# ubc-vision/UniT

Measured on AMD Instinct MI355X. Metric: images/sec (fwd+bwd+SGD) R101-C4 VOC 600x1000 bs=2/GPU, higher is better.
Workload: dtype bf16; 1 GPU; UniT base-training step S1 (TrainerNoMeta.run_step): ResNet-101-C4, VOC split1 K=20, 2 supervised + 2 weak 3x600x1000 images per GPU, 512 RoIs/image, two Res5 heads, RPN 12000->2000, all 8 losses, SGD momentum; images_per_gpu=2, global_batch=2, parallelism=dp1

## Files before the change

include/unit_hip.h:

```cpp
#ifndef UNIT_HIP_H
#define UNIT_HIP_H
#include <stddef.h>
#include <stdint.h>
#ifdef __cplusplus
extern "C" {
#endif

int unit_version(void);
const char* unit_build_hash(void);
const char* unit_last_error(void);

int unit_preprocess_image(const float* img_chw, int C, int H, int W, const float* mean3, const float* std3, float prescale,
                          void* out_nhwc, int out_dtype, int Hmax, int Wmax, int Cpad, void* stream);
int unit_resize_u8_pass(const unsigned char* src, int H, int W, int C, int axis, const int* bounds, const int* kk, int ksize,
                        int out_size, unsigned char* dst, void* stream);
int unit_preprocess_u8(const unsigned char* img_hwc, int C, int H, int W, int hflip, const float* mean3, const float* std3,
                       float prescale, void* out_nhwc, int out_dtype, int Hmax, int Wmax, int Cpad, void* stream);
int unit_nchw_to_nhwc(const float* x, void* y, int dtype, int N, int C, int H, int W, int Cp, void* stream);
int unit_nhwc_to_nchw(const void* x, int dtype, float* y, int N, int C, int H, int W, int Cp, void* stream);
int unit_debug_spin(long long cycles, void* sink, void* stream);
int unit_cast(const void* x, int in_dtype, void* y, int out_dtype, long n, void* stream);
int unit_fill_zero(void* p, size_t nbytes, void* stream);
int unit_add_cast(const float* a32, const void* b, const void* mask_ref, void* y, int dtype, long n, void* stream);

// ... 25 lines not shown
                        int N, int H, int W, int C, int K, int R, int S, int stride, int pad, int OH, int OW, int ldy, int oy_mul, int OHf,
                        int OWf, int relu, int tile, int segs, void* stream);
int unit_conv2d_wgrad_x3(const void* x, const void* dy, float* dw, const float* scale_k, int N, int H, int W, int C, int K, int R, int S,
                         int stride, int pad, int OH, int OW, int ldy, int accumulate, int variant, void* workspace, size_t workspace_bytes,
                         void* stream);
int unit_global_avgpool_x3_fwd(const void* y, float* out, int R, int rows, int C, void* stream);
int unit_global_avgpool_x3_bwd_relu(const float* dfeat, const void* y, void* g, int R, int rows, int C, void* stream);
typedef struct UnitConvSecond {
  const void* x; void* y; const void* residual; const void* mask_ref;
  int N, H, W, OHf, OWf;
} UnitConvSecond;
int unit_conv2d_fwd_pair(int kernel, const void* x, const void* w, void* y, const float* bias, const void* residual, const void* mask_ref, int mask_c,
                         int in_dtype, int out_dtype, int N, int H, int W, int C, int K, int R, int S, int stride, int pad, int OH, int OW, int ldy,
                         int oy_mul, int OHf, int OWf, int relu, int tile, const UnitConvSecond* second, void* stream);
size_t unit_conv2d_wgrad_workspace_bytes(int in_dtype, int N, int OH, int OW, int K, int R, int S, int C);
int unit_conv2d_wgrad(const void* x, const void* dy, float* dw, const float* scale_k, int in_dtype, int N, int H, int W, int C,
                      int K, int R, int S, int stride, int pad, int OH, int OW, int ldy, int accumulate, int variant, void* workspace,
                      size_t workspace_bytes, void* stream);
int unit_conv2d_wgrad_splits(int in_dtype, int N, int OH, int OW, int K, int R, int S, int C);
typedef struct UnitWgradProblem {
  const void* x; const void* dy; void* partial;
  int N, H, W, C, K, R, S, stride, pad, OH, OW, ldy;
  int splits, kind;
  int x_pitch;
  int x_back, dy_back;
} UnitWgradProblem;
size_t unit_wgrad_problem_bytes(void);
int unit_conv2d_wgrad_group_supported(int in_dtype, int N, int OH, int OW, int K, int R, int S, int C);
int unit_conv2d_wgrad_group_plan(UnitWgradProblem* pr, int n, int splits_hint);
int unit_conv2d_wgrad_group(const UnitWgradProblem* pr, int n, int in_dtype, void* stream);
int unit_conv2d_wgrad_group_layout(const UnitWgradProblem* pr, int n, int* layout, int layout_rows, int* rows);
int unit_stream_wait_stream(void* waiter, void* signaller);
size_t unit_tensor_desc_bytes(void);
int unit_multi_wgrad_reduce(const void* descs_dev, int n, int total_blocks, float* grads_flat, void* stream);
int unit_multi_weight_prep(const void* descs_dev, int n, int total_blocks, const float* params_flat, int dtype, void* stream);
int unit_shard_sum(const void* parts, int dtype, int nparts, long n, float* out, void* stream);
int unit_comm_unique_id(void* id, int id_bytes);
int unit_comm_init(int rank, int world, const void* id, int id_bytes, void** comm);
int unit_allreduce_bucket_async(void* comm, void* buf, long count, int dtype, void* stream);
int unit_comm_wait(void* compute_stream, void* comm_stream);
int unit_comm_destroy(void* comm);
int unit_comm_rccl_version(void);
int unit_frozen_bn_fold(const float* w, const float* b, const float* rm, const float* rv, float eps, float* scale, float* shift,
                        int C, void* stream);
int unit_weight_prep(const float* w_krsc, const float* scale_k, int K, int R, int S, int C, int Cp, void* w_fwd, void* w_dgrad,
                     int dtype, void* stream);
size_t unit_bias_grad_scratch_bytes(int M, int K);
int unit_bias_grad(const void* dy, int dtype, int M, int K, int ld, float* db, int accumulate, float* scratch, size_t scratch_bytes,
                   void* stream);
size_t unit_linear_wgrad_workspace_bytes(int R, int C, int K);
int unit_linear_wgrad(const void* x, const void* dy, int dtype, int R, int C, int K, int ldy, float* dw, float* db,
                      void* workspace, size_t workspace_bytes, void* stream);
int unit_stem_conv_pool(const void* x, const void* w, const float* shift, void* y, int dtype, int N, int H, int W, void* stream);
int unit_maxpool3x3s2_fwd(const void* x, void* y, int dtype, int N, int H, int W, int C, void* stream);
int unit_global_avgpool_fwd(const void* x, void* y, int dtype, int R, int P, int C, void* stream);
int unit_global_avgpool_bwd_relu(const void* dfeat, const void* out, void* g, int dtype, int R, int P, int C, void* stream);

int unit_anchor_grid(float* out, int H, int W, int A, float stride, float offset, const float* cell_dev, void* stream);

size_t unit_iou_match_workspace_bytes(int B, int Mcap);
int unit_iou_match(const float* gt, const int* gt_count, int B, int Mcap, const float* boxes, long box_batch_stride,
                   const int* box_count, int Ncap, const float* thresholds, const int* labels, int n_thresh,
                   int allow_low_quality, int64_t* match_idx, int8_t* match_label, float* match_val, void* workspace,
                   size_t workspace_bytes, void* stream);
int unit_pairwise_iou(const float* b1, int M, const float* b2, int Nb, float* out, void* stream);
int unit_match_matrix(const float* q, int M, int N, const float* thresholds, const int* labels, int n_thresh, int allow_low_quality,
                      int64_t* match_idx, int8_t* match_label, float* match_val, float* rowmax_ws, void* stream);

int unit_subsample_labels(const void* labels, int labels_are_int64, const int* count, int B, int Ncap, const int* perm, int Pcap,
                          int num_samples, int max_pos, int bg_label, int8_t* out_labels, int* sampled_idx, int* out_counts,
                          void* stream);

int unit_box_encode(const float* src, const float* tgt, const float* weights4, float* out, int n, void* stream);
int unit_box_decode(const float* deltas, int ld, int col0, int K, const float* boxes, const float* weights4, float scale_clamp,
                    float* out, int n, void* stream);

size_t unit_sort_workspace_bytes(int B, int n);
int unit_sort_desc_stable(const float* src, long batch_stride, int ld, int A, int col0, int B, int n, float* out_keys, int* out_idx,
                          void* workspace, size_t workspace_bytes, void* stream);
int unit_sort_desc_stable_topk(const float* src, long batch_stride, int ld, int A, int col0, int B, int n, int topk,
                               float min_exclusive, float* out_keys, int* out_idx, void* workspace, size_t workspace_bytes,
                               void* stream);
int unit_rpn_decode_select(const float* head, long head_batch_stride, int ld, int A, int delta_col0, const float* anchors,
                           const int* sorted_idx, const float* sorted_logit, int B, int Ncap, int topk, const float* image_hw_dev,
                           float scale_clamp, float min_size, float* cand_boxes, float* cand_scores, int* cand_count, void* stream);
size_t unit_nms_workspace_bytes(int B, int cap);
int unit_nms(const float* boxes_sorted, const float* scores_sorted, const int* count, int B, int cap, float thresh, int max_keep,
             int* keep_idx, int* keep_count, float* out_boxes, float* out_scores, void* workspace, size_t workspace_bytes,
             void* stream);

int unit_append_gt(const float* props, const int* pcount, int Pcap, const float* gt, const int* gcount, int Mcap, int B, float* cat,
                   int* ccount, void* stream);
int unit_roi_classes(const int64_t* match_idx, const int8_t* match_label, const int* count, const int64_t* gt_classes,
                     const int* gcount, int Mcap, int B, int Ncap, int K, int64_t* cls, void* stream);
int unit_gather_rois(const float* cat, int Ncap, const int* sampled_idx, int S, const int64_t* cls, const int64_t* match_idx,
                     const float* gt, const int* gcount, int Mcap, int B, float* rois, int* roi_cls, float* roi_gt, void* stream);
int unit_first_k_rois(const float* props, const int* pcount, int Pcap, int S, int B, int batch_index_offset, float* rois, int* valid,
                      void* stream);

int unit_roi_align_fwd(const void* feat_nhwc, int dtype, int N, int H, int W, int C, const float* rois, const int* roi_count_dev,
                       int R, int pooled_size, int out_size, int bin_step, float spatial_scale, int sampling_ratio, int aligned,
                       void* out, void* stream);
int unit_roi_align_bwd(const void* gout, int dtype, int N, int H, int W, int C, const float* rois, const int* roi_count_dev, int R,
                       int pooled_size, int out_size, int bin_step, float spatial_scale, int sampling_ratio, int aligned,
                       float* dfeat_f32, void* stream);

// ... 102 lines not shown
```

unit_amd/build.py:

```python
import hashlib
import os
import subprocess
import sys
from concurrent.futures import ThreadPoolExecutor

HERE = os.path.dirname(os.path.abspath(__file__))
CSRC = os.path.join(HERE, "csrc")
OUT_DIR = os.path.join(HERE, "_build")
LIB = os.path.join(OUT_DIR, "libunit_hip.so")
HEADER = os.path.join(os.path.dirname(HERE), "include", "unit_hip.h")
SOURCES = ["elementwise.hip", "input_pipeline.hip", "boxes.hip", "sort_nms.hip", "roi_align.hip", "losses.hip", "pcl.hip", "conv_igemm.hip", "conv_igemm256.hip", "conv_igemm256p8.hip", "conv_igemm256p8m.hip", "conv_igemm128.hip", "conv_igemm_lc.hip", "conv_wgrad.hip", "conv_wgrad256.hip", "conv_wgrad256p8.hip", "conv_wgrad256r.hip", "conv_wgrad128r.hip", "linear_wgrad.hip", "stem_pool.hip", "detect.hip", "mask.hip", "multi.hip", "split.hip", "comm.hip", "replay.hip"]
STAMP = "build_stamp.hip"
FLAGS = ["--offload-arch=gfx950", "-O3", "-fPIC", "-ffp-contract=off", "-std=c++17", "-Wno-unused-value"]


def _hipcc():
    for c in ("/opt/rocm/bin/hipcc", "hipcc"):
        if os.path.exists(c) or c == "hipcc":
            return c
    return "hipcc"


def _read(path):
    with open(path, "rb") as f:
        return f.read()


def _headers():
    return sorted(os.path.join(CSRC, f) for f in os.listdir(CSRC) if f.endswith(".h"))


def _digest(paths, extra=()):
    h = hashlib.sha256()
    for e in extra:
        h.update(str(e).encode() + b"\0")
    for p in paths:
        h.update(os.path.basename(p).encode() + b"\0")
        h.update(_read(p))
        h.update(b"\0")
    return h.hexdigest()


def source_hash():
    srcs = [os.path.join(CSRC, s) for s in SOURCES + [STAMP]]
    return _digest(srcs + _headers() + [HEADER], extra=FLAGS)


def _stamp_of(path):
    try:
        with open(path + ".hash") as f:
            return f.read().strip()
    except OSError:
        return None


def _write_stamp(path, digest):
    with open(path + ".hash", "w") as f:
        f.write(digest + "\n")


def build(force=False, verbose=False):
    os.makedirs(OUT_DIR, exist_ok=True)
    hdrs = _headers()
    want = source_hash()
# ... 33 lines not shown
```

unit_amd/layers.py:

```python
import os

import torch
from torch import nn

from . import ops


_FROZEN_EPOCH = [0]


def invalidate_prepared():
    _FROZEN_EPOCH[0] += 1


class _EpochOnLoad(nn.Module):
    def _load_from_state_dict(self, *args, **kwargs):
        invalidate_prepared()
        return super()._load_from_state_dict(*args, **kwargs)


def _krsc_storage(w):
    if w.dim() == 2:
        return w if w.is_contiguous() else w.contiguous()
    k, c, r, s = w.shape
# ... 201 lines not shown
            ops.bias_grad(dy_plain.reshape(-1, dy_plain.shape[-1]), self.cout, out=self.bias.grad, accumulate=acc)


def set_x3(module, on):
    n = 0
    for m in module.modules():
        if isinstance(m, Conv2d):
            ok = bool(on) and m.cin % 64 == 0 and m.cout % 64 == 0 and m.cin_pad == m.cin and not getattr(m, "_in_linear_group", False)
            if ok != m.x3:
                m.x3 = ok
                m._prep_key = None
            n += int(ok)
    return n


class BottleneckBlock(nn.Module):

    def __init__(self, cin, cout, bottleneck, stride):
        super().__init__()
        self.stride = stride
        self.shortcut = Conv2d(cin, cout, 1, stride, 0, norm=True) if cin != cout else None
        self.conv1 = Conv2d(cin, bottleneck, 1, stride, 0, norm=True)
        self.conv2 = Conv2d(bottleneck, bottleneck, 3, 1, 1, norm=True)
        self.conv3 = Conv2d(bottleneck, cout, 1, 1, 0, norm=True)

    def convs(self):
        return [c for c in (self.conv1, self.conv2, self.conv3, self.shortcut) if c is not None]

    def fwd(self, x, save=False, stride=None, pool_rows=0, x_bits=None, out_bits=False, pooled_out=None):
        st = self.stride if stride is None else stride
        if isinstance(x, ops.Ragged):
            if self.conv1.x3 and type(x.flat) is not ops.X3:
                x = x.like(ops.x3_split(x.flat))
        elif self.conv1.x3:
            x = ops.as_x3(x)
        y1 = self.conv1.fwd(x, relu=True, stride=st)
        y2 = self.conv2.fwd(y1, relu=True)
        if self._dual_ok(x, y2, st) and not pool_rows:
            wcat, bcat = self._cat_weights("fwd")
            out, bits, _ = ops.conv2d_ex(y2, wcat, self.conv3.cout, 1, 1, 0, bias=bcat, relu=True, want_bits=out_bits, x2=x)
            return ((out, bits) if out_bits else out), ((x, y1, y2, st, x_bits) if save else None)
        sc = self.shortcut.fwd(x, stride=st) if self.shortcut is not None else x
        if pool_rows:
            c3 = self.conv3
            _, bits, pooled = ops.conv2d_ex(y2, c3.wf, c3.cout, 1, 1, 0, bias=c3.shift, residual=sc, relu=True, want_bits=save,
                                            pool_rows=pool_rows, want_y=False, pooled_out=pooled_out)
            return (pooled, bits), ((x, y1, y2, st, x_bits) if save else None)
        if out_bits:
            c3 = self.conv3
            out, bits, _ = ops.conv2d_ex(y2, c3.wf, c3.cout, 1, 1, 0, bias=c3.shift, residual=sc, relu=True, want_bits=True)
            return (out, bits), ((x, y1, y2, st, x_bits) if save else None)
        out = self.conv3.fwd(y2, relu=True, residual=sc)
        return out, ((x, y1, y2, st, x_bits) if save else None)

    def _dual_ok(self, x, y2, st):
        if isinstance(x, ops.Ragged):
            return False
        return (ops.FUSE_EPILOGUE and ops.FUSE_DUAL and getattr(self, "allow_dual", False) and self.shortcut is not None and st == 1
                and x.dtype == torch.bfloat16 and x.shape[:3] == y2.shape[:3] and x.shape[0] > 0
                and ops.conv_ex_supported(x.dtype, self.conv3.cin, self.conv3.cout) and self.shortcut.cin % self.conv3.cin == 0
                and self.shortcut.cout % self.conv1.cout == 0 and self.conv1.cout % 64 == 0 and self.conv1.cin % 64 == 0)

    def prepare_dual(self):
        if not (ops.FUSE_EPILOGUE and ops.FUSE_DUAL and getattr(self, "allow_dual", False) and self.shortcut is not None):
            return
        c3, sc, c1 = self.conv3, self.shortcut, self.conv1
        if c3.x3 or sc.x3 or c1.x3:
            return
        if c3.wf is None or sc.wf is None or c3.wf.dtype != torch.bfloat16 or c3.k != 1 or sc.k != 1 or c1.k != 1:
            return
        key = (c3.wf.data_ptr(), sc.wf.data_ptr(), 0 if c1.wd is None else c1.wd.data_ptr(), 0 if sc.wd is None else sc.wd.data_ptr(),
               0 if c3.shift is None else c3.shift.data_ptr(), 0 if sc.shift is None else sc.shift.data_ptr())
        if self.__dict__.get("_dual_key") == key:
            return
        dev, dt = c3.wf.device, c3.wf.dtype
        buf = torch.empty((c3.cout, 1, 1, c3.cin + sc.cin), dtype=dt, device=dev)
        v = buf.view(c3.cout, -1)
        c3.link_copy("wf", v[:, :c3.cin])
        sc.link_copy("wf", v[:, c3.cin:])
        self.__dict__["_wcat_fwd"] = buf
        self.__dict__["_wcat_bwd"] = None
        if c1.wd is not None and sc.wd is not None:
            bufb = torch.empty((c1.cin, 1, 1, c1.cout + sc.cout), dtype=dt, device=dev)
            vb = bufb.view(c1.cin, -1)
            c1.link_copy("wd", vb[:, :c1.cout])
            sc.link_copy("wd", vb[:, c1.cout:])
            self.__dict__["_wcat_bwd"] = bufb
        self.__dict__["_bcat"] = c3.shift + sc.shift
        self.__dict__["_dual_key"] = key

    def _cat_weights(self, which):
        self.prepare_dual()
        buf = self.__dict__.get("_wcat_" + which)
        assert buf is not None, "dual-input GEMM before the block's weights were prepared"
        return buf, (self.__dict__["_bcat"] if which == "fwd" else None)

    def bwd(self, ctx, g, need_dx=True, mask_input=True):
        x, y1, y2, st, x_bits = ctx
        rag = isinstance(x, ops.Ragged)
        if rag:
            if self.conv3.x3 and type(g.flat) is not ops.X3:
                g = g.like(ops.x3_split(g.flat))
        elif self.conv3.x3:
            g = ops.as_x3(g)
        hw_of = (lambda t: t.dims) if rag else (lambda t: t.shape[1:3])
        self.conv3.wgrad(y2, g)
        dy2 = self.conv3.dgrad(g, hw_of(y2), mask_ref=y2)
        self.conv2.wgrad(y1, dy2)
        dy1 = self.conv2.dgrad(dy2, hw_of(y1), mask_ref=y1)
        self.conv1.wgrad(x, dy1, stride=st)
        if self.shortcut is not None:
            self.shortcut.wgrad(x, g, stride=st)
        if not need_dx:
            return None
        hw = hw_of(x)
        if self._dual_ok(x, y2, st) and not mask_input and g.dtype == torch.bfloat16:
            wcat, _ = self._cat_weights("bwd")
            return ops.conv2d_ex(dy1, wcat, self.conv1.cin, 1, 1, 0, x2=g)[0]
        if self.shortcut is not None:
            dsc = self.shortcut.dgrad(g, hw, stride=st)
        else:
            dsc = g
        return self.conv1.dgrad(dy1, hw, mask_ref=x if mask_input else None, residual=dsc, stride=st, mask_bits=x_bits if mask_input else None)


class ResStage(nn.Sequential):
    def __init__(self, num_blocks, cin, cout, bottleneck, first_stride):
        blocks = [BottleneckBlock(cin if i == 0 else cout, cout, bottleneck, first_stride if i == 0 else 1) for i in range(num_blocks)]
        super().__init__(*blocks)

    def fwd(self, x, save=False, first_stride=None, pool_rows=0, out_bits=False, pooled_out=None):
        ctxs = []
        x_bits = None
        for i, b in enumerate(self):
            last = i == len(self) - 1
            ob = (out_bits and not last and not isinstance(x, ops.Ragged) and ops.conv_ex_supported(x.dtype, b.conv3.cin, b.conv3.cout)
                  and (i > 0 or (first_stride or b.stride) == 1))
            x, c = b.fwd(x, save, stride=first_stride if i == 0 else None, pool_rows=pool_rows if last else 0, x_bits=x_bits, out_bits=ob,
                         pooled_out=pooled_out if last else None)
            x_bits = None
            if ob:
                x, x_bits = x
            ctxs.append(c)
        return x, ctxs

    def bwd(self, ctxs, g, need_dx=True, mask_input=True, on_block_done=None):
        n = len(self)
        for i in range(n - 1, -1, -1):
            first = i == 0
            g = self[i].bwd(ctxs[i], g, need_dx=(need_dx or not first), mask_input=(mask_input or not first))
            if on_block_done is not None:
                on_block_done(i)
        return g

    BUCKET_BLOCKS = 6

    def bucket_of_block(self, i):
        n = len(self)
        if n <= self.BUCKET_BLOCKS + 2:
            return 0
        return (n - 1 - i) // self.BUCKET_BLOCKS

    def last_block_of_bucket(self, k):
        n = len(self)
        if n <= self.BUCKET_BLOCKS + 2:
            return 0
        return max(0, n - (k + 1) * self.BUCKET_BLOCKS)


_FUSED_STEM = os.environ.get("UNIT_FUSED_STEM", "1") != "0"


class BasicStem(nn.Module):

    def __init__(self, cout=64):
        super().__init__()
        self.conv1 = Conv2d(3, cout, 7, 2, 3, norm=True, cin_pad=8)

    def fwd(self, x):
        c = self.conv1
        if isinstance(x, (list, tuple)):
            dims = []
            for t in x:
                n, h, w, _ = t.shape
                oh, ow = (h - 1) // 2 + 1, (w - 1) // 2 + 1
                dims.append((n, (oh - 1) // 2 + 1, (ow - 1) // 2 + 1))
            out = ops.Ragged.empty(dims, c.cout, x[0])
            for i, t in enumerate(x):
                self._fwd_one(t, out.group(i))
            return out
        return self._fwd_one(x, None)

    def _fwd_one(self, x, out):
        c = self.conv1
        if (_FUSED_STEM and x.dtype == torch.bfloat16 and x.is_cuda and c.cout == 64 and x.shape[-1] == 8 and c.wf is not None
                and c.wf.dtype == torch.bfloat16 and not c.weight.requires_grad):
            return ops.stem_conv_pool(x, c.wf, c.shift, out=out)
# ... 122 lines not shown
```

unit_amd/modeling/backbone.py:

```python
import os

import torch
from torch import nn

from .. import ops
from ..layers import BasicStem, ResStage
from ..structures import BACKBONE_REGISTRY, ShapeSpec

BLOCKS = {50: [3, 4, 6, 3], 101: [3, 4, 23, 3], 152: [3, 8, 36, 3]}


class ResNet(nn.Module):
    def __init__(self, depth=101, freeze_at=2, res2_out=256, width=64):
        super().__init__()
        nb = BLOCKS[depth]
        self.depth = depth
        self.stem = BasicStem(64)
        self.res2 = ResStage(nb[0], 64, res2_out, width, 1)
        self.res3 = ResStage(nb[1], res2_out, res2_out * 2, width * 2, 2)
        self.res4 = ResStage(nb[2], res2_out * 2, res2_out * 4, width * 4, 2)
        self.out_channels = res2_out * 4
        self.size_divisibility = 0
        self.freeze_at = freeze_at
        self.freeze(freeze_at)

    def freeze(self, freeze_at):
        stages = [self.stem, self.res2, self.res3, self.res4]
        for i, s in enumerate(stages, start=1):
            if freeze_at >= i:
                for p in s.parameters():
                    p.requires_grad = False
        self.res2[0].allow_dual = freeze_at >= 2 and os.environ.get("UNIT_RES2_DUAL", "0") == "1"
        return self

    def output_shape(self):
        return {"res4": ShapeSpec(channels=self.out_channels, stride=16)}

    def all_convs(self):
        cs = [self.stem.conv1]
        for st in (self.res2, self.res3, self.res4):
            for b in st:
                cs += b.convs()
        return cs

    def prepare(self, dtype, version):
        for c in self.all_convs():
            c.prepare(dtype, version, need_dgrad=c.weight.requires_grad)

    def first_trainable_stage(self):
        for i, st in enumerate((self.res2, self.res3, self.res4)):
            if any(p.requires_grad for p in st.parameters()):
                return i
        return 3

    def fwd(self, x, save=False, before_trainable=None):
        joined = False
        if before_trainable is not None and any(p.requires_grad for p in self.stem.parameters()):
            before_trainable()
            joined = True
        x = self.stem.fwd(x)
        ft = self.first_trainable_stage()
        ctx = []
        for i, st in enumerate((self.res2, self.res3, self.res4)):
            if i == ft and before_trainable is not None and not joined:
                before_trainable()
            x, c = st.fwd(x, save=save and i >= ft)
            ctx.append(c)
        return x, ctx

    def bwd(self, ctx, g, on_stage_done=None):
        ft = self.first_trainable_stage()
        stages = (self.res2, self.res3, self.res4)
        for i in (2, 1, 0):
            if i < ft:
                break
            name, st = ("res2", "res3", "res4")[i], stages[i]
            cb = None
            if on_stage_done is not None:
                def cb(j, name=name, st=st):
                    k = st.bucket_of_block(j)
                    if j == st.last_block_of_bucket(k):
                        on_stage_done(name if k == 0 else f"{name}.{k}")
            g = st.bwd(ctx[i], g, need_dx=(i > ft), mask_input=True, on_block_done=cb)
        return None

    def forward(self, x):
        if self.training and torch.is_grad_enabled():
            from .train_modules import backbone_forward_train
            return backbone_forward_train(self, x)
        dtype = getattr(self, "compute_dtype", torch.bfloat16)
        self.prepare(dtype, 0)
        xh = ops.nchw_to_nhwc(x, dtype=dtype, cpad=8)
        y, _ = self.fwd(xh)
        return {"res4": ops.nhwc_to_nchw(y)}


@BACKBONE_REGISTRY.register()
def build_resnet_backbone(cfg, input_shape=None):
    r = cfg.MODEL.RESNETS
    assert r.NORM == "FrozenBN" and r.STRIDE_IN_1X1 and r.NUM_GROUPS == 1, "C4 hot path: FrozenBN, stride_in_1x1, groups=1"
    assert list(r.OUT_FEATURES) == ["res4"]
    return ResNet(r.DEPTH, cfg.MODEL.BACKBONE.FREEZE_AT, r.RES2_OUT_CHANNELS, r.WIDTH_PER_GROUP)
```

unit_amd/ops.py:

```python
import ctypes
import os
import math

import torch

from ._lib import _DEBUG_SYNC, check, lib

F32, BF16 = 0, 1
SCALE_CLAMP = math.log(1000.0 / 16)


def dt(dtype):
    if dtype == torch.float32:
        return F32
    if dtype == torch.bfloat16:
        return BF16
    raise TypeError(f"unsupported dtype {dtype}")


def _p(t):
    if t is None:
        return None
    if not t.is_cuda:
        raise RuntimeError("unit_amd ops need tensors on the ROCm device (no CPU fallback)")
# ... 352 lines not shown
            out = zeros((n, ohf, owf, ldy), out_dtype, x.device)
        else:
            out = torch.empty((n, ohf, owf, ldy), dtype=out_dtype, device=x.device)
    prof = PROFILER
    if prof is not None:
        e0 = torch.cuda.Event(enable_timing=True)
        e0.record()
    big, mid, variant = False, -1, 0
    if tile_cfg == 0:
        pkey = (x.dtype, n * oh * ow, k, c, r * s * c, out_dtype, ldy % 8, BIG_TILE_POLICY, MID_TILE_POLICY)
        pol = _POLICY_CACHE.get(pkey)
        if pol is None:
            pol = _POLICY_CACHE[pkey] = select_conv_kernel(x.dtype, n * oh * ow, k, c, r * s * c, out_dtype, ldy)
        big, mid = pol
    elif tile_cfg >= 100:
        mid = tile_cfg
    elif tile_cfg in TILE_CFG:
        kind, code = TILE_CFG[tile_cfg]
        if kind == "big":
            big, variant = True, code
        else:
            mid = code
    if mid >= 0:
        check(lib().unit_conv2d_fwd_mid(_p(x), _p(w), _p(out), _p(bias), _p(residual), _p(mask_ref), dt(out_dtype),
                                        n, h, wd, c, k, r, s, stride, pad, oh, ow, ldy, oy_mul, ohf, owf, int(relu), mid, _s()),
              "unit_conv2d_fwd_mid")
    elif big:
        check(lib().unit_conv2d_fwd_big(_p(x), _p(w), _p(out), _p(bias), _p(residual), _p(mask_ref), dt(out_dtype),
                                        n, h, wd, c, k, r, s, stride, pad, oh, ow, ldy, oy_mul, ohf, owf, int(relu),
                                        variant, _s()),
              "unit_conv2d_fwd_big")
    else:
        check(lib().unit_conv2d_fwd(_p(x), _p(w), _p(out), _p(bias), _p(residual), _p(mask_ref), dt(x.dtype), dt(out_dtype),
                                    n, h, wd, c, k, r, s, stride, pad, oh, ow, ldy, oy_mul, ohf, owf, int(relu), tile_cfg, _s()),
              "unit_conv2d_fwd")
    if prof is not None:
        e1 = torch.cuda.Event(enable_timing=True)
        e1.record()
        es = out.element_size()
        nbytes = (x.numel() + w.numel()) * x.element_size() + n * oh * ow * ldy * es * (1 + (residual is not None) + (mask_ref is not None))
        feed = None
        if mid >= 0:
            bm, bn = mid_tile_dims(mid)
            tiles = ((n * oh * ow + bm - 1) // bm) * ((k + bn - 1) // bn)
            feed = ((tiles + 255) // 256) * (r * s * c // 64) * (bm + bn) * 128.0
        prof.setdefault("conv_igemm256" if (big and mid < 0) else ("conv_igemm_dma" if mid >= 0 else "conv_igemm"), []).append(
            (e0, e1, 2.0 * n * oh * ow * k * r * s * c, nbytes, feed))
    return out


FUSE_EPILOGUE = os.environ.get("UNIT_FUSE_EPILOGUE", "1") != "0"


FUSE_DUAL = os.environ.get("UNIT_FUSE_DUAL", "1") != "0"


def conv_ex_supported(dtype, c, ldy):
    return dtype == torch.bfloat16 and c % 64 == 0 and ldy % 64 == 0


class ReluBits:

    def __init__(self, data, r, bins, c, roi0=0):
        self.data, self.r, self.bins, self.c, self.roi0 = data, r, bins, c, roi0

    def __getitem__(self, sl):
        start, stop, step = sl.indices(self.r)
        assert step == 1
        return ReluBits(self.data, stop - start, self.bins, self.c, self.roi0 + start)

    def aligned(self):
        m0 = self.roi0 * self.bins
        if m0 % 128:
            return None
        return self if m0 == 0 else ReluBits(self.data[(m0 // 128) * (self.c // 64) * 1024:], self.r, self.bins, self.c, 0)

    def unpack(self):
        dev = self.data.device
        m = torch.arange(self.roi0 * self.bins, (self.roi0 + self.r) * self.bins, device=dev).view(-1, 1)
        n = torch.arange(self.c, device=dev).view(1, -1)
        word = ((m >> 7) * (self.c >> 6) + (n >> 6)) * 64 + ((m & 7) * 8 + ((n & 63) >> 3))
        byte = self.data[word * 16 + ((m & 127) >> 3)]
        return ((byte.int() >> (n & 7)) & 1).bool().view(self.r, self.bins, self.c)


def conv2d_ex(x, w, k, r, s, pad=0, bias=None, residual=None, relu=False, mask_bits=None, want_bits=False, pool_rows=0, want_y=True, x2=None, variant=0,
              pooled_out=None):
    n, h, wd, c = x.shape
    c2 = 0
    if x2 is not None:
        c2 = x2.shape[3]
        assert r == 1 and s == 1 and pad == 0 and x2.shape[:3] == x.shape[:3] and c2 % c == 0 and x2.dtype == x.dtype and w.shape[-1] == c + c2
    oh, ow = conv_out_size(h, wd, r, s, 1, pad)
    ldy = k
    assert conv_ex_supported(x.dtype, c, ldy), "conv2d_ex: bf16, C % 64 == 0, K % 8 == 0"
    m = n * oh * ow
    y = torch.empty((n, oh, ow, ldy), dtype=x.dtype, device=x.device) if want_y else None
    bits = None
    if want_bits:
        bits = ReluBits(torch.empty(lib().unit_relu_bits_bytes(m, ldy), dtype=torch.uint8, device=x.device), n, oh * ow, k)
    if mask_bits is not None:
        assert mask_bits.roi0 == 0 and mask_bits.r * mask_bits.bins == m and mask_bits.c == k
    part = None
    if pool_rows:
        assert pool_rows == oh * ow
        part = torch.empty(lib().unit_conv_pool_partial_floats(m, ldy), dtype=torch.float32, device=x.device)
# ... 417 lines not shown
def frozen_bn_fold(weight, bias, running_mean, running_var, eps=1e-5):
    c = weight.numel()
    scale = torch.empty(c, dtype=torch.float32, device=weight.device)
    shift = torch.empty(c, dtype=torch.float32, device=weight.device)
    check(lib().unit_frozen_bn_fold(_p(weight), _p(bias), _p(running_mean), _p(running_var), eps, _p(scale), _p(shift), c, _s()),
          "frozen_bn_fold")
    return scale, shift


def weight_prep(w_krsc, scale, k, r, s, c, cp, dtype, want_dgrad=True, w_fwd=None, w_dgrad=None):
    dev = w_krsc.device
    if w_fwd is None:
        w_fwd = torch.empty((k, r, s, cp), dtype=dtype, device=dev)
    if want_dgrad and w_dgrad is None:
        w_dgrad = torch.empty((c, r, s, k), dtype=dtype, device=dev)
    check(lib().unit_weight_prep(_p(w_krsc), _p(scale), k, r, s, c, cp, _p(w_fwd), _p(w_dgrad) if want_dgrad else None,
                                 dt(dtype), _s()), "weight_prep")
    return w_fwd, w_dgrad


def bias_grad(dy2d, k, out=None, accumulate=False):
    m, ld = dy2d.shape
    if out is None:
        out = torch.empty(k, dtype=torch.float32, device=dy2d.device)
    nb = lib().unit_bias_grad_scratch_bytes(m, k) if m > 1024 else 0
    ws = workspace(nb, dy2d.device, slot=3) if nb else None
    check(lib().unit_bias_grad(_p(dy2d), dt(dy2d.dtype), m, k, ld, _p(out), int(accumulate), _p(ws), nb, _s()), "bias_grad")
    return out


def linear_wgrad(x2d, dy2d, k, dw, db):
    r, c = x2d.shape
    ldy = dy2d.shape[1]
    dev = x2d.device
    nb = lib().unit_linear_wgrad_workspace_bytes(r, c, k)
    ws = workspace(nb, dev, slot=4)
    with _timed("conv_wgrad", 2.0 * r * k * c, (x2d.numel() + r * ldy) * 2 + 4 * k * c):
        check(lib().unit_linear_wgrad(_p(x2d), _p(dy2d), dt(x2d.dtype), r, c, k, ldy, _p(dw), _p(db), _p(ws), ws.numel(), _s()),
              "unit_linear_wgrad")


def stem_conv_pool(x, w_fwd, shift, out=None):
    n, h, w, c = x.shape
    assert c == 8 and tuple(w_fwd.shape) == (64, 7, 7, 8) and x.dtype == torch.bfloat16 and w_fwd.dtype == torch.bfloat16
    oh, ow = (h - 1) // 2 + 1, (w - 1) // 2 + 1
    ph, pw = (oh - 1) // 2 + 1, (ow - 1) // 2 + 1
    y = out if out is not None else torch.empty((n, ph, pw, 64), dtype=x.dtype, device=x.device)
    assert tuple(y.shape) == (n, ph, pw, 64) and y.is_contiguous()
    with _timed("stem", 2.0 * n * oh * ow * 64 * 147, x.numel() * 2 + y.numel() * 2):
        check(lib().unit_stem_conv_pool(_p(x), _p(w_fwd), _p(shift), _p(y), dt(x.dtype), n, h, w, _s()), "unit_stem_conv_pool")
    return y


def maxpool3x3s2(x, out=None):
    n, h, w, c = x.shape
    oh, ow = (h + 2 - 3) // 2 + 1, (w + 2 - 3) // 2 + 1
    y = out if out is not None else torch.empty((n, oh, ow, c), dtype=x.dtype, device=x.device)
    assert tuple(y.shape) == (n, oh, ow, c) and y.is_contiguous() and y.dtype == x.dtype
    check(lib().unit_maxpool3x3s2_fwd(_p(x), _p(y), dt(x.dtype), n, h, w, c, _s()), "maxpool")
    return y


def global_avgpool(x, out=None):
    r, ph, pw, c = x.shape
    if out is not None:
        assert out.shape == (r, c) and out.is_contiguous() and out.dtype == (torch.float32 if type(x) is X3 else x.dtype)
    if type(x) is X3:
        y = out if out is not None else torch.empty((r, c), dtype=torch.float32, device=x.device)
        check(lib().unit_global_avgpool_x3_fwd(_px(x), _p(y), r, ph * pw, c, _s()), "avgpool_x3_fwd")
        return y
    y = out if out is not None else torch.empty((r, c), dtype=x.dtype, device=x.device)
    check(lib().unit_global_avgpool_fwd(_p(x), _p(y), dt(x.dtype), r, ph * pw, c, _s()), "avgpool_fwd")
    return y


def global_avgpool_bwd_relu(dfeat, out):
    r, ph, pw, c = out.shape
    if type(out) is X3:
        g = torch.empty(out.shape, dtype=torch.float32, device=out.device).as_subclass(X3)
        check(lib().unit_global_avgpool_x3_bwd_relu(_p(dfeat), _px(out), _px(g), r, ph * pw, c, _s()), "avgpool_x3_bwd")
        return g
    g = torch.empty_like(out)
    check(lib().unit_global_avgpool_bwd_relu(_p(dfeat), _p(out), _p(g), dt(out.dtype), r, ph * pw, c, _s()), "avgpool_bwd")
    return g


def cell_anchors(sizes=(32, 64, 128, 256, 512), ratios=(0.5, 1.0, 2.0)):
    out = []
    for size in sizes:
        area = size ** 2.0
        for r in ratios:
            w = math.sqrt(area / r)
            h = r * w
            out.append([-w / 2.0, -h / 2.0, w / 2.0, h / 2.0])
    return torch.tensor(out, dtype=torch.float32)


def anchor_grid(h, w, cell, stride=16, offset=0.0):
    a = cell.shape[0]
    out = torch.empty((h * w * a, 4), dtype=torch.float32, device=cell.device)
    check(lib().unit_anchor_grid(_p(out), h, w, a, float(stride), float(offset), _p(cell), _s()), "anchor_grid")
    return out


def iou_match(gt, gt_count, boxes, box_count, thresholds, labels, allow_low_quality, want_vals=True):
    b, mcap = gt.shape[0], gt.shape[1]
# ... 452 lines not shown
```

Baseline: 132.6 images/sec.

## Fuse frozen res2 bottleneck blocks into one persistent HIP kernel

Adds a kernel that runs a whole frozen res2 bottleneck block (1x1, 3x3, 1x1, plus the optional shortcut conv, with bias, residual and ReLU) per spatial tile in LDS. Weights stay in registers, and the next tile is prefetched with buffer-load-to-LDS. When the next stage begins with a stride-2 1x1 conv, the last block writes only the pixels that consumer reads. This removes the intermediate activation round-trips to HBM and the per-conv launches in the frozen res2 stage. In exchange it recomputes halo pixels for conv1, and the stride-2 output leaves the other pixels unwritten, so correctness depends on no other consumer reading them.

Measured after the change: 131.6 images/sec, median of 2. Within noise of the previous version (-0.7%).

```diff
diff --git a/include/unit_hip.h b/include/unit_hip.h
--- a/include/unit_hip.h
+++ b/include/unit_hip.h
@@ -101,6 +101,8 @@
 int unit_linear_wgrad(const void* x, const void* dy, int dtype, int R, int C, int K, int ldy, float* dw, float* db,
                       void* workspace, size_t workspace_bytes, void* stream);
 int unit_stem_conv_pool(const void* x, const void* w, const float* shift, void* y, int dtype, int N, int H, int W, void* stream);
+int unit_res2_block_fwd(const void* x, const void* w1, const float* b1, const void* w2, const float* b2, const void* w3, const float* b3,
+                        const void* wsc, const float* bsc, void* y, int N, int H, int W, int cin, int out_stride, void* stream);
 int unit_maxpool3x3s2_fwd(const void* x, void* y, int dtype, int N, int H, int W, int C, void* stream);
 int unit_global_avgpool_fwd(const void* x, void* y, int dtype, int R, int P, int C, void* stream);
 int unit_global_avgpool_bwd_relu(const void* dfeat, const void* out, void* g, int dtype, int R, int P, int C, void* stream);
diff --git a/unit_amd/build.py b/unit_amd/build.py
--- a/unit_amd/build.py
+++ b/unit_amd/build.py
@@ -9,7 +9,7 @@
 OUT_DIR = os.path.join(HERE, "_build")
 LIB = os.path.join(OUT_DIR, "libunit_hip.so")
 HEADER = os.path.join(os.path.dirname(HERE), "include", "unit_hip.h")
-SOURCES = ["elementwise.hip", "input_pipeline.hip", "boxes.hip", "sort_nms.hip", "roi_align.hip", "losses.hip", "pcl.hip", "conv_igemm.hip", "conv_igemm256.hip", "conv_igemm256p8.hip", "conv_igemm256p8m.hip", "conv_igemm128.hip", "conv_igemm_lc.hip", "conv_wgrad.hip", "conv_wgrad256.hip", "conv_wgrad256p8.hip", "conv_wgrad256r.hip", "conv_wgrad128r.hip", "linear_wgrad.hip", "stem_pool.hip", "detect.hip", "mask.hip", "multi.hip", "split.hip", "comm.hip", "replay.hip"]
+SOURCES = ["elementwise.hip", "input_pipeline.hip", "boxes.hip", "sort_nms.hip", "roi_align.hip", "losses.hip", "pcl.hip", "conv_igemm.hip", "conv_igemm256.hip", "conv_igemm256p8.hip", "conv_igemm256p8m.hip", "conv_igemm128.hip", "conv_igemm_lc.hip", "conv_wgrad.hip", "conv_wgrad256.hip", "conv_wgrad256p8.hip", "conv_wgrad256r.hip", "conv_wgrad128r.hip", "linear_wgrad.hip", "stem_pool.hip", "res2_block.hip", "detect.hip", "mask.hip", "multi.hip", "split.hip", "comm.hip", "replay.hip"]
 STAMP = "build_stamp.hip"
 FLAGS = ["--offload-arch=gfx950", "-O3", "-fPIC", "-ffp-contract=off", "-std=c++17", "-Wno-unused-value"]
 
diff --git a/unit_amd/csrc/res2_block.hip b/unit_amd/csrc/res2_block.hip
--- /dev/null
+++ b/unit_amd/csrc/res2_block.hip
@@ -0,0 +1,314 @@
+#include "common.h"
+#include "conv_epilogue.h"
+#ifndef UNIT_RES2_DBG
+#define UNIT_RES2_DBG 0
+#endif
+
+namespace {
+
+typedef __attribute__((address_space(3))) void lds_void_r;
+
+constexpr int TH = 4, TW = 16;
+constexpr int NW = 4;
+constexpr int NA = 256 / NW / 16;
+constexpr int PW = TW + 2;
+constexpr int PPIX = (TH + 2) * PW;
+constexpr int PROWS = (PPIX + 15) / 16 * 16;
+constexpr int PBLK = PROWS / 16, PPIECES = PROWS / 8;
+constexpr int PLANE = PROWS * 128;
+constexpr int Y2_BYTES = TH * TW * 128;
+constexpr int OPLANE_SC = TH * TW * 128;
+
+template <bool SC> struct Lds {
+  static constexpr int NPL = SC ? 1 : 4;
+  static constexpr int Y1 = NPL * PLANE, Y2 = Y1 + PLANE;
+  static constexpr int OUT = SC ? Y2 + Y2_BYTES : 0;
+  static constexpr int SHIFT = SC ? OUT + 4 * OPLANE_SC : Y2 + Y2_BYTES;
+  static constexpr int BYTES = SHIFT + (SC ? 2048 : 1024);
+};
+static_assert(2 * Lds<true>::BYTES <= 160 * 1024 && 2 * Lds<false>::BYTES <= 160 * 1024, "LDS budget: two workgroups per CU");
+
+struct Res2Args {
+  const bf16_t* x; const bf16_t* w1; const bf16_t* w2; const bf16_t* w3; const bf16_t* wsc;
+  const float* b1; const float* b2; const float* b3; const float* bsc;
+  bf16_t* y;
+  int N, H, W, tiles_x, tiles_y, ntiles, per_xcd;
+  unsigned x_bytes;
+};
+
+__device__ __forceinline__ int swz_r(int row, int chunk) { return row * 128 + ((chunk ^ ((row >> 1) & 7)) << 4); }
+
+__device__ __forceinline__ bf16x8 ldw(const bf16_t* w, int row, int pitch, int k) {
+  return __builtin_bit_cast(bf16x8, *reinterpret_cast<const i32x4*>(w + (size_t)row * pitch + k));
+}
+
+template <bool RELU, bool RES>
+__device__ __forceinline__ i32x2 finish4(const f32x4& acc, const float (&b)[4], i32x2 res) {
+  float v[4];
+#pragma unroll
+  for (int j = 0; j < 4; ++j) v[j] = acc[j] + b[j];
+  if constexpr (RES) {
+    v[0] += epi_lo((unsigned)res[0]); v[1] += epi_hi((unsigned)res[0]);
+    v[2] += epi_lo((unsigned)res[1]); v[3] += epi_hi((unsigned)res[1]);
+  }
+  unsigned o0 = epi_cvt_pk(v[0], v[1]), o1 = epi_cvt_pk(v[2], v[3]);
+  if constexpr (RELU) { o0 = epi_relu_pk(o0); o1 = epi_relu_pk(o1); }
+  return i32x2{(int)o0, (int)o1};
+}
+
+template <bool SC, int OS>
+__global__ void __launch_bounds__(NW * 64, 2) res2_block_kernel(Res2Args p) {
+  typedef Lds<SC> L;
+  constexpr int CIN = SC ? 64 : 256;
+  constexpr int KS1 = CIN / 32;
+  constexpr int NPT = TH * TW / (OS * OS) / 16;
+  constexpr int NCP = NPT * 16 * 32 / (NW * 64);
+  extern __shared__ __attribute__((aligned(16))) char smem[];
+  char* const xs = smem;
+  char* const y1 = smem + L::Y1;
+  char* const y2 = smem + L::Y2;
+  char* const outs = smem + L::OUT;
+  float* const shifts = reinterpret_cast<float*>(smem + L::SHIFT);
+
+  const int tid = threadIdx.x, lane = tid & 63;
+  const int wid = __builtin_amdgcn_readfirstlane(tid >> 6);
+  const int frow = lane & 15, fq = lane >> 4;
+  const int sl = wid;
+  const int lrow = lane >> 3, lc = lane & 7;
+
+  __amdgpu_buffer_rsrc_t rsX = __builtin_amdgcn_make_buffer_rsrc(const_cast<bf16_t*>(p.x), 0, (int)p.x_bytes, 0x00020000);
+  constexpr unsigned OOB = 0xFFFFFFF0u;
+
+  const int xcd = blockIdx.x & 7, loc0 = blockIdx.x >> 3, wg_per_xcd = gridDim.x >> 3;
+  auto tile_of = [&](int loc) { int t = xcd * p.per_xcd + loc; return (loc < p.per_xcd && t < p.ntiles) ? t : -1; };
+
+  bool staged = false;
+  auto stage = [&](int tile) {
+    int tx = tile % p.tiles_x, t2 = tile / p.tiles_x, ty = t2 % p.tiles_y, n = t2 / p.tiles_y;
+    int py0 = ty * TH - 1, px0 = tx * TW - 1;
+    if ((UNIT_RES2_DBG & 1) && staged) return;
+    staged = true;
+#pragma unroll
+    for (int i = 0; i < (L::NPL * PPIECES + NW - 1) / NW; ++i) {
+      int pc = wid + NW * i;
+      if (pc >= L::NPL * PPIECES) break;
+      int pl = pc / PPIECES, R0 = (pc - pl * PPIECES) * 8;
+      int row = R0 + lrow;
+      int q = lc ^ ((row >> 1) & 7);
+      int py = row / PW, px = row - py * PW;
+      int yy = py0 + py, xx = px0 + px;
+      bool ok = row < PPIX && (unsigned)yy < (unsigned)p.H && (unsigned)xx < (unsigned)p.W;
+      unsigned off = ((unsigned)((n * p.H + yy) * p.W + xx) * (unsigned)CIN + (unsigned)(pl * 64 + q * 8)) * 2u;
+      __builtin_amdgcn_raw_ptr_buffer_load_lds(rsX, (lds_void_r*)(xs + pl * PLANE + R0 * 128), 16, ok ? off : OOB, 0, 0, 0);
+    }
+  };
+
+  int loc = loc0;
+  int tile = tile_of(loc);
+  if (tile >= 0) stage(tile);
+
+  bf16x8 fw1[KS1], fw2[9][2], fw3[NA][2], fws[SC ? NA : 1][2];
+  float bb1[4], bb2[4];
+  static_assert(NW * 64 == 256, "one thread per output channel");
+  shifts[tid] = p.b3[tid];
+  if constexpr (SC) shifts[256 + tid] = p.bsc[tid];
+#pragma unroll
+  for (int j = 0; j < KS1; ++j) fw1[j] = ldw(p.w1, sl * 16 + frow, CIN, j * 32 + fq * 8);
+#pragma unroll
+  for (int t = 0; t < 9; ++t)
+#pragma unroll
+    for (int ks = 0; ks < 2; ++ks) fw2[t][ks] = ldw(p.w2, sl * 16 + frow, 576, t * 64 + ks * 32 + fq * 8);
+#pragma unroll
+  for (int a = 0; a < NA; ++a)
+#pragma unroll
+    for (int ks = 0; ks < 2; ++ks) {
+      fw3[a][ks] = ldw(p.w3, wid * (NA * 16) + a * 16 + frow, 64, ks * 32 + fq * 8);
+      if constexpr (SC) fws[a][ks] = ldw(p.wsc, wid * (NA * 16) + a * 16 + frow, 64, ks * 32 + fq * 8);
+    }
+#pragma unroll
+  for (int j = 0; j < 4; ++j) {
+    bb1[j] = p.b1[sl * 16 + fq * 4 + j];
+    bb2[j] = p.b2[sl * 16 + fq * 4 + j];
+  }
+  auto shift4 = [&](const float* b, int a, float (&v)[4]) {
+    f32x4 t = *reinterpret_cast<const f32x4*>(b + wid * (NA * 16) + a * 16 + fq * 4);
+    v[0] = t[0]; v[1] = t[1]; v[2] = t[2]; v[3] = t[3];
+  };
+
+  auto out_pos = [](int j, int& py, int& px) {
+    if constexpr (OS == 1) { py = j >> 4; px = j & 15; }
+    else { py = (j >> 3) * 2; px = (j & 7) * 2; }
+  };
+
+  while (tile >= 0) {
+    const int tx = tile % p.tiles_x, t2 = tile / p.tiles_x, ty = t2 % p.tiles_y, n = t2 / p.tiles_y;
+    const int y0 = ty * TH, x0 = tx * TW;
+    asm volatile("s_waitcnt vmcnt(0)" ::: "memory");
+    __syncthreads();
+
+    if (!(UNIT_RES2_DBG & 2)) {
+#pragma unroll 1
+    for (int rt = 0; rt < PBLK; ++rt) {
+      const int row = rt * 16 + frow;
+      f32x4 acc = {0.f, 0.f, 0.f, 0.f};
+      bf16x8 fx[KS1];
+#pragma unroll
+      for (int j = 0; j < KS1; ++j) fx[j] = *reinterpret_cast<const bf16x8*>(xs + (j >> 1) * PLANE + swz_r(row, (j & 1) * 4 + fq));
+#pragma unroll
+      for (int j = 0; j < KS1; ++j) acc = __builtin_amdgcn_mfma_f32_16x16x32_bf16(fw1[j], fx[j], acc, 0, 0, 0);
+      int py = row / PW, px = row - py * PW;
+      bool in_map = row < PPIX && (unsigned)(y0 - 1 + py) < (unsigned)p.H && (unsigned)(x0 - 1 + px) < (unsigned)p.W;
+      i32x2 o = finish4<true, false>(acc, bb1, i32x2{0, 0});
+      if (!in_map) o = i32x2{0, 0};
+      const int ch = sl * 16 + fq * 4;
+      *reinterpret_cast<i32x2*>(y1 + swz_r(row, ch >> 3) + (ch & 4) * 2) = o;
+    }
+    }
+    __syncthreads();
+
+    if (!(UNIT_RES2_DBG & 2)) {
+#pragma unroll 1
+    for (int i = 0; i < NPT; ++i) {
+      const int j0 = i * 16;
+      int py, px;
+      out_pos(j0 + frow, py, px);
+      f32x4 acc = {0.f, 0.f, 0.f, 0.f};
+#pragma unroll
+      for (int r = 0; r < 3; ++r) {
+        bf16x8 fx[3][2];
+#pragma unroll
+        for (int s = 0; s < 3; ++s)
+#pragma unroll
+          for (int ks = 0; ks < 2; ++ks) fx[s][ks] = *reinterpret_cast<const bf16x8*>(y1 + swz_r((py + r) * PW + px + s, ks * 4 + fq));
+#pragma unroll
+        for (int s = 0; s < 3; ++s)
+#pragma unroll
+          for (int ks = 0; ks < 2; ++ks) acc = __builtin_amdgcn_mfma_f32_16x16x32_bf16(fw2[r * 3 + s][ks], fx[s][ks], acc, 0, 0, 0);
+      }
+      i32x2 o = finish4<true, false>(acc, bb2, i32x2{0, 0});
+      const int ch = sl * 16 + fq * 4;
+      *reinterpret_cast<i32x2*>(y2 + swz_r(j0 + frow, ch >> 3) + (ch & 4) * 2) = o;
+    }
+    }
+    __syncthreads();
+
+    if (!(UNIT_RES2_DBG & 2)) {
+#pragma unroll 1
+    for (int pt = 0; pt < NPT; ++pt) {
+      const int j = pt * 16 + frow;
+      int py, px;
+      out_pos(j, py, px);
+      const int prow = (py + 1) * PW + px + 1;
+      bf16x8 f2[2];
+#pragma unroll
+      for (int ks = 0; ks < 2; ++ks) f2[ks] = *reinterpret_cast<const bf16x8*>(y2 + swz_r(j, ks * 4 + fq));
+      f32x4 acc[NA];
+#pragma unroll
+      for (int a = 0; a < NA; ++a) acc[a] = f32x4{0.f, 0.f, 0.f, 0.f};
+#pragma unroll
+      for (int a = 0; a < NA; ++a)
+#pragma unroll
+        for (int ks = 0; ks < 2; ++ks) acc[a] = __builtin_amdgcn_mfma_f32_16x16x32_bf16(fw3[a][ks], f2[ks], acc[a], 0, 0, 0);
+      i32x2 res[NA];
+      if constexpr (SC) {
+        bf16x8 fxs[2];
+#pragma unroll
+        for (int ks = 0; ks < 2; ++ks) fxs[ks] = *reinterpret_cast<const bf16x8*>(xs + swz_r(prow, ks * 4 + fq));
+#pragma unroll
+        for (int a = 0; a < NA; ++a) {
+          f32x4 as = {0.f, 0.f, 0.f, 0.f};
+#pragma unroll
+          for (int ks = 0; ks < 2; ++ks) as = __builtin_amdgcn_mfma_f32_16x16x32_bf16(fws[a][ks], fxs[ks], as, 0, 0, 0);
+          float bs[4];
+          shift4(shifts + 256, a, bs);
+          res[a] = finish4<false, false>(as, bs, i32x2{0, 0});
+        }
+      }
+#pragma unroll
+      for (int a = 0; a < NA; ++a) {
+        const int ch = wid * (NA * 16) + a * 16 + fq * 4;
+        const int orow = SC ? j : prow;
+        char* q = outs + (ch >> 6) * (SC ? OPLANE_SC : PLANE) + swz_r(orow, (ch & 63) >> 3) + (ch & 4) * 2;
+        if constexpr (!SC) res[a] = *reinterpret_cast<const i32x2*>(q);
+        float b3[4];
+        shift4(shifts, a, b3);
+        *reinterpret_cast<i32x2*>(q) = finish4<true, true>(acc[a], b3, res[a]);
+      }
+    }
+    }
+    __syncthreads();
+
+    loc += wg_per_xcd;
+    const int next = tile_of(loc);
+    constexpr int NH = NCP / 2;
+    i32x4 ov[NH];
+    auto take = [&](int k0) {
+#pragma unroll
+      for (int k = 0; k < NH; ++k) {
+        int item = tid + NW * 64 * (k0 + k);
+        int j = item >> 5, c = item & 31;
+        int py, px;
+        out_pos(j, py, px);
+        const int orow = SC ? j : (py + 1) * PW + px + 1;
+        ov[k] = *reinterpret_cast<const i32x4*>(outs + (c >> 3) * (SC ? OPLANE_SC : PLANE) + swz_r(orow, c & 7));
+      }
+    };
+    auto put = [&](int k0) {
+#pragma unroll
+      for (int k = 0; k < NH; ++k) {
+        int item = tid + NW * 64 * (k0 + k);
+        int j = item >> 5, c = item & 31;
+        int py, px;
+        out_pos(j, py, px);
+        int yy = y0 + py, xx = x0 + px;
+        if (yy < p.H && xx < p.W && (!(UNIT_RES2_DBG & 4) || ov[k][0] == 0x7fc17fc3))
+          *reinterpret_cast<i32x4*>(p.y + (((size_t)n * p.H + yy) * p.W + xx) * 256 + c * 8) = ov[k];
+      }
+    };
+    take(0);
+    put(0);
+    take(NH);
+    if constexpr (!SC) __syncthreads();
+    if (next >= 0) stage(next);
+    put(NH);
+    tile = next;
+  }
+}
+
+template <bool SC, int OS>
+int launch_res2(const Res2Args& a, hipStream_t st) {
+  static bool attr_set = false;
+  if (!attr_set) {
+    (void)hipFuncSetAttribute((const void*)res2_block_kernel<SC, OS>, hipFuncAttributeMaxDynamicSharedMemorySize, Lds<SC>::BYTES);
+    attr_set = true;
+  }
+  int grid = a.ntiles < 512 ? (a.ntiles + 7) / 8 * 8 : 512;
+  res2_block_kernel<SC, OS><<<grid, NW * 64, Lds<SC>::BYTES, st>>>(a);
+  UNIT_LAUNCH_CHECK();
+  return UNIT_OK;
+}
+
+}
+
+extern "C" int unit_res2_block_fwd(const void* x, const void* w1, const float* b1, const void* w2, const float* b2, const void* w3,
+                                   const float* b3, const void* wsc, const float* bsc, void* y, int N, int H, int W, int cin, int out_stride,
+                                   void* stream) {
+  UNIT_CHECK_ARG(x && w1 && b1 && w2 && b2 && w3 && b3 && y, "unit_res2_block_fwd: null tensor");
+  UNIT_CHECK_ARG((wsc != nullptr) == (bsc != nullptr), "unit_res2_block_fwd: shortcut weights and shift come together");
+  UNIT_CHECK_ARG(cin == (wsc ? 64 : 256), "unit_res2_block_fwd: 64 input channels with a shortcut conv, 256 without");
+  UNIT_CHECK_ARG(out_stride == 1 || out_stride == 2, "unit_res2_block_fwd: out_stride must be 1 or 2");
+  UNIT_CHECK_ARG(N > 0 && H > 0 && W > 0 && (size_t)N * H * W * 256 * 2 < 0xFFFFFFF0ull, "unit_res2_block_fwd: bad shape");
+  UNIT_CHECK_ARG(((uintptr_t)x % 16 == 0) && ((uintptr_t)y % 16 == 0) && ((uintptr_t)w1 % 16 == 0) && ((uintptr_t)w2 % 16 == 0) &&
+                 ((uintptr_t)w3 % 16 == 0) && ((uintptr_t)wsc % 16 == 0), "unit_res2_block_fwd: 16B alignment");
+  Res2Args a;
+  a.x = (const bf16_t*)x; a.w1 = (const bf16_t*)w1; a.w2 = (const bf16_t*)w2; a.w3 = (const bf16_t*)w3; a.wsc = (const bf16_t*)wsc;
+  a.b1 = b1; a.b2 = b2; a.b3 = b3; a.bsc = bsc; a.y = (bf16_t*)y;
+  a.N = N; a.H = H; a.W = W;
+  a.tiles_x = cdiv(W, TW); a.tiles_y = cdiv(H, TH);
+  a.ntiles = a.tiles_x * a.tiles_y * N;
+  a.per_xcd = cdiv(a.ntiles, 8);
+  a.x_bytes = (unsigned)((size_t)N * H * W * cin * 2);
+  hipStream_t st = (hipStream_t)stream;
+  if (wsc) return out_stride == 1 ? launch_res2<true, 1>(a, st) : launch_res2<true, 2>(a, st);
+  return out_stride == 1 ? launch_res2<false, 1>(a, st) : launch_res2<false, 2>(a, st);
+}
diff --git a/unit_amd/layers.py b/unit_amd/layers.py
--- a/unit_amd/layers.py
+++ b/unit_amd/layers.py
@@ -277,6 +277,21 @@
             return (out, bits), ((x, y1, y2, st, x_bits) if save else None)
         out = self.conv3.fwd(y2, relu=True, residual=sc)
         return out, ((x, y1, y2, st, x_bits) if save else None)
+
+    def fused_frozen_ok(self, cin):
+        c1, c2, c3, sc = self.conv1, self.conv2, self.conv3, self.shortcut
+        if self.stride != 1 or getattr(self, "allow_dual", False) or any(p.requires_grad for p in self.parameters()):
+            return False
+        if any(c.x3 or c.wf is None or c.wf.dtype != torch.bfloat16 or c.shift is None or c.cin_pad != c.cin for c in self.convs()):
+            return False
+        if (c1.k, c1.cin, c1.cout, c2.k, c2.pad, c2.cin, c2.cout, c3.k, c3.cin, c3.cout) != (1, cin, 64, 3, 1, 64, 64, 1, 64, 256):
+            return False
+        return cin == 256 if sc is None else (cin == 64 and (sc.k, sc.cin, sc.cout) == (1, 64, 256))
+
+    def fwd_frozen_fused(self, x, out_stride=1):
+        c1, c2, c3, sc = self.conv1, self.conv2, self.conv3, self.shortcut
+        return ops.res2_block_fwd(x, c1.wf, c1.shift, c2.wf, c2.shift, c3.wf, c3.shift, sc.wf if sc is not None else None,
+                                  sc.shift if sc is not None else None, out_stride=out_stride)
 
     def _dual_ok(self, x, y2, st):
         if isinstance(x, ops.Ragged):
@@ -368,6 +383,21 @@
                 x, x_bits = x
             ctxs.append(c)
         return x, ctxs
+
+    def fused_frozen_ok(self, x):
+        if not ops.FUSE_RES2 or not isinstance(x, torch.Tensor) or type(x) is ops.X3 or x.dtype != torch.bfloat16 or x.dim() != 4 or x.shape[0] == 0:
+            return False
+        cin = x.shape[3]
+        for b in self:
+            if not b.fused_frozen_ok(cin):
+                return False
+            cin = b.conv3.cout
+        return True
+
+    def fwd_frozen_fused(self, x, consumer_stride=1):
+        for i, b in enumerate(self):
+            x = b.fwd_frozen_fused(x, out_stride=consumer_stride if i == len(self) - 1 else 1)
+        return x, [None] * len(self)
 
     def bwd(self, ctxs, g, need_dx=True, mask_input=True, on_block_done=None):
         n = len(self)
diff --git a/unit_amd/modeling/backbone.py b/unit_amd/modeling/backbone.py
--- a/unit_amd/modeling/backbone.py
+++ b/unit_amd/modeling/backbone.py
@@ -64,9 +64,20 @@
         for i, st in enumerate((self.res2, self.res3, self.res4)):
             if i == ft and before_trainable is not None and not joined:
                 before_trainable()
-            x, c = st.fwd(x, save=save and i >= ft)
+            if i < ft and st.fused_frozen_ok(x):
+                x, c = st.fwd_frozen_fused(x, consumer_stride=self._consumer_stride(i))
+            else:
+                x, c = st.fwd(x, save=save and i >= ft)
             ctx.append(c)
         return x, ctx
+
+    def _consumer_stride(self, i):
+        stages = (self.res2, self.res3, self.res4)
+        if i + 1 >= len(stages):
+            return 1
+        b = stages[i + 1][0]
+        ok = (b.stride == 2 and b.shortcut is not None and all((c.k, c.pad, c.stride) == (1, 0, 2) for c in (b.conv1, b.shortcut)))
+        return 2 if ok else 1
 
     def bwd(self, ctx, g, on_stage_done=None):
         ft = self.first_trainable_stage()
diff --git a/unit_amd/ops.py b/unit_amd/ops.py
--- a/unit_amd/ops.py
+++ b/unit_amd/ops.py
@@ -428,6 +428,7 @@
 FUSE_EPILOGUE = os.environ.get("UNIT_FUSE_EPILOGUE", "1") != "0"
 
 
+FUSE_RES2 = os.environ.get("UNIT_FUSE_RES2", "1") != "0"
 FUSE_DUAL = os.environ.get("UNIT_FUSE_DUAL", "1") != "0"
 
 
@@ -951,6 +952,24 @@
     return y
 
 
+def res2_block_fwd(x, w1, b1, w2, b2, w3, b3, wsc=None, bsc=None, out=None, out_stride=1):
+    n, h, w, c = x.shape
+    assert x.dtype == torch.bfloat16 and x.is_contiguous() and c == (64 if wsc is not None else 256)
+    assert tuple(w1.shape) == (64, 1, 1, c) and tuple(w2.shape) == (64, 3, 3, 64) and tuple(w3.shape) == (256, 1, 1, 64)
+    assert wsc is None or tuple(wsc.shape) == (256, 1, 1, 64)
+    assert all(t is None or (t.dtype == torch.bfloat16 and t.is_contiguous()) for t in (w1, w2, w3, wsc))
+    assert all(t is None or (t.dtype == torch.float32 and t.is_contiguous()) for t in (b1, b2, b3, bsc))
+    y = out if out is not None else torch.empty((n, h, w, 256), dtype=x.dtype, device=x.device)
+    assert tuple(y.shape) == (n, h, w, 256) and y.is_contiguous() and y.dtype == x.dtype
+    m = n * h * w
+    mo = m if out_stride == 1 else n * ((h + 1) // 2) * ((w + 1) // 2)
+    flops = 2.0 * (m * 64 * c + mo * (576 * 64 + 64 * 256 * (2 if wsc is not None else 1)))
+    with _timed("res2_block", flops, x.numel() * 2 + mo * 256 * 2):
+        check(lib().unit_res2_block_fwd(_p(x), _p(w1), _p(b1), _p(w2), _p(b2), _p(w3), _p(b3), _p(wsc), _p(bsc), _p(y), n, h, w, c,
+                                        int(out_stride), _s()), "unit_res2_block_fwd")
+    return y
+
+
 def maxpool3x3s2(x, out=None):
     n, h, w, c = x.shape
     oh, ow = (h + 2 - 3) // 2 + 1, (w + 2 - 3) // 2 + 1
```
